# twosixlabs/csl-gan

Measured on AMD Instinct MI355X. Metric: images/sec/GPU CelebA DCResNet dp_mode=gc bs=128 at 1/2/4/8 MI355X, higher is better.
Workload: dtype f32; 1 GPU; CelebA DCResNet D-step: dp_mode=gc -gcm adaptive-pl -nms 32, WGAN-GP on mean samples, 3x64x64; compute_dtype=fp32_auto, storage_dtype=fp32, launch=hip_graph, batch_per_gpu=128, global_batch=128, parallelism=dp1, materialize=ghost, grad_sample_dtype=fp32, fuse_passes=True

## Files before the change

### csl_gan_amd/_lib.py

```python
from __future__ import annotations

import ctypes as C
import os

_HERE = os.path.dirname(os.path.abspath(__file__))
LIB_PATH = os.environ.get("CSLGAN_LIB_PATH") or os.path.join(_HERE, "libcslgan_hip.so")
MAX_SEGS = 16
ABI_VERSION = 7

EXPORTS = [
    "cslgan_version", "cslgan_last_error", "cslgan_last_kernel", "cslgan_device_count",
    "cslgan_sample_sqnorm_f32", "cslgan_sample_sqnorm_bf16", "cslgan_clip_factors_f32", "cslgan_clip_accum_noise_f32",
    "cslgan_clip_accum_noise_bf16", "cslgan_conv2d_wgrad_grouped_bf16out_f32",
    "cslgan_l2_clip_rows_f32", "cslgan_row_l2norm_f32", "cslgan_row_l2norm_bwd_f32", "cslgan_mean_sample_f32",
    "cslgan_conv2d_fwd_f32", "cslgan_conv2d_fwd_x3_f32", "cslgan_conv2d_dgrad_f32", "cslgan_conv2d_wgrad_grouped_f32",
    "cslgan_conv2d_wgrad_scaled_f32", "cslgan_conv2d_wgrad_blocks_f32", "cslgan_conv2d_wgrad_sqnorm_gram_f32", "cslgan_conv2d_wgrad_skinny_f32", "cslgan_conv2d_s2_fwd_f32",
    "cslgan_conv2d_dgrad_x3_f32", "cslgan_conv2d_s2_fwd_x3_f32", "cslgan_u8_to_f32_nhwc", "cslgan_split_filter_x3_f32",
    "cslgan_depth_to_space_f32", "cslgan_fold_channels4_f32",
    "cslgan_bias_grad_grouped_f32", "cslgan_act_bwd_f32", "cslgan_groupnorm_act_f32", "cslgan_groupnorm_apply_parts_f32", "cslgan_groupnorm_apply_parts_shortcut_f32", "cslgan_groupnorm_affine_parts_f32", "cslgan_batchnorm_act_f32", "cslgan_batchnorm_eval_act_f32",
    "cslgan_norm_act_bwd_f32", "cslgan_norm_bwd_ws_floats",
    "cslgan_adam_step_f32", "cslgan_adam_step_dev_f32", "cslgan_adam_multi_f32",
    "cslgan_adaptive_clip_f32", "cslgan_segment_means_f32", "cslgan_segment_means_bwd_f32", "cslgan_dstep_stats_f32", "cslgan_grad_log_stats_f32",
    "cslgan_lerp_rows_f32", "cslgan_lipschitz_term_f32", "cslgan_lipschitz_term_bwd_f32",
    "cslgan_conv2d_fwd_bf16s", "cslgan_conv2d_dgrad_bf16s", "cslgan_conv2d_wgrad_grouped_bf16s", "cslgan_cast_f32_bf16", "cslgan_cast_bf16_f32",
    "cslgan_act_bwd_bf16", "cslgan_bias_grad_grouped_bf16", "cslgan_linear_k1_dgrad_bf16s", "cslgan_linear_k1_wgrad_bf16s",
    "cslgan_conv2d_c3_fwd_bf16out", "cslgan_conv2d_c3_wgrad_bf16gy", "cslgan_groupnorm_act_bf16s",
    "cslgan_conv2d_fwd_skinny_bf16in", "cslgan_conv2d_dgrad_skinny_bf16in", "cslgan_conv2d_wgrad_scaled_bf16s",
    "cslgan_latent_normal_f32", "cslgan_f32_to_u8",
    "cslgan_attack_trials", "cslgan_rank_counts", "cslgan_softmax_max_rows_f32",
    "cslgan_ovr_logreg_ws_floats", "cslgan_ovr_logreg_eval_f32", "cslgan_ovr_logreg_proba_f32",
    "cslgan_ovr_logreg_u8_ws_floats", "cslgan_ovr_logreg_eval_u8", "cslgan_ovr_logreg_proba_u8",
    "cslgan_ovr_mlp_u8_ws_floats", "cslgan_ovr_mlp_eval_u8", "cslgan_ovr_mlp_proba_u8",
    "cslgan_class_moments_u8", "cslgan_nb_score_gauss_u8", "cslgan_nb_score_bern_u8",
    "cslgan_tree_best_split_ws_bytes", "cslgan_tree_best_split_u8", "cslgan_tree_apply_u8",
    "cslgan_boost_stump_ws_bytes", "cslgan_boost_stump_u8",
    "cslgan_nn_padded_dim", "cslgan_nn_prepare_u8", "cslgan_nn_min_i8", "cslgan_nn_count_i8",
    "cslgan_nn_kth_workspace_bytes", "cslgan_nn_kth_i8", "cslgan_nn_count_radius_i8",
    "cslgan_gram_d2_u8", "cslgan_svc_smo_f64",
    "cslgan_swd_directions_i8", "cslgan_swd_project_i8", "cslgan_sort_rows_ws_bytes", "cslgan_sort_rows_i32", "cslgan_swd_w1_i64",
]


class SegsT(C.Structure):
    _fields_ = [
        ("n_seg", C.c_int32), ("_pad", C.c_int32),
        ("inp", C.c_void_p * MAX_SEGS), ("out", C.c_void_p * MAX_SEGS), ("noise", C.c_void_p * MAX_SEGS),
        ("len", C.c_int64 * MAX_SEGS), ("row_stride", C.c_int64 * MAX_SEGS), ("rows", C.c_int64 * MAX_SEGS), ("call_counter", C.c_void_p),
    ]


MAX_CLIP_LAYERS, MAX_CLIP_JOBS = 32, 16


class AdaptiveClipT(C.Structure):
    _fields_ = [
        ("n_layers", C.c_int32), ("n_mat", C.c_int32), ("n_jobs", C.c_int32), ("_pad", C.c_int32),
        ("sq_adapt", C.c_void_p * MAX_CLIP_LAYERS), ("sq_rows", C.c_void_p * MAX_CLIP_LAYERS), ("mat_layer", C.c_int32 * MAX_CLIP_LAYERS),
        ("job_dst", C.c_void_p * MAX_CLIP_JOBS), ("job_first", C.c_int64 * MAX_CLIP_JOBS), ("job_layer", C.c_int32 * MAX_CLIP_JOBS),
        ("job_count", C.c_int32 * MAX_CLIP_JOBS), ("job_scale", C.c_float * MAX_CLIP_JOBS),
    ]


class ConvT(C.Structure):
    _fields_ = [(n, C.c_int32) for n in
                ("N", "H", "W", "C", "K", "R", "S", "stride", "pad", "compute", "P", "Q")] + [("split_ws", C.c_void_p), ("split_ws_floats", C.c_int64), ("gn_part", C.c_void_p), ("gn_groups", C.c_int32), ("in_relu", C.c_int32), ("in_scale", C.c_void_p), ("in_shift", C.c_void_p)]


_lib = None


class HipLibraryMissing(RuntimeError):
    pass


def lib():
    global _lib
    if _lib is not None:
        return _lib
    if not os.path.exists(LIB_PATH):
        raise HipLibraryMissing(
# ... 18 lines not shown
        "cslgan_row_l2norm_f32": [vp, i64, i64, vp, vp],
        "cslgan_row_l2norm_bwd_f32": [vp, vp, vp, i64, i64, vp, vp],
        "cslgan_conv2d_fwd_f32": [C.POINTER(ConvT), vp, vp, vp, vp, i32, vp, vp],
        "cslgan_conv2d_fwd_x3_f32": [C.POINTER(ConvT), vp, vp, vp, i32, vp, vp, i32, vp, vp],
        "cslgan_conv2d_dgrad_f32": [C.POINTER(ConvT), vp, vp, vp, i32, vp, vp, vp],
        "cslgan_conv2d_dgrad_x3_f32": [C.POINTER(ConvT), vp, vp, vp, vp, i32, vp, vp, vp],
        "cslgan_norm_act_bwd_f32": [vp, vp, vp, vp, vp, i64, i64, i32, i32, f32, i32, vp, vp, vp, vp, vp],
        "cslgan_depth_to_space_f32": [vp, i32, i32, i32, i32, i32, vp, vp],
        "cslgan_fold_channels4_f32": [vp, i64, i32, i32, vp, vp],
        "cslgan_conv2d_wgrad_grouped_f32": [C.POINTER(ConvT), vp, vp, i32, f32, vp, vp, vp],
        "cslgan_conv2d_wgrad_scaled_f32": [C.POINTER(ConvT), vp, vp, vp, i32, f32, vp, vp],
        "cslgan_conv2d_wgrad_blocks_f32": [C.POINTER(ConvT), vp, vp, f32, i32, C.POINTER(C.c_int32), C.POINTER(vp), C.POINTER(vp), vp],
        "cslgan_conv2d_wgrad_sqnorm_gram_f32": [C.POINTER(ConvT), vp, vp, f32, vp, vp],
        "cslgan_conv2d_wgrad_skinny_f32": [C.POINTER(ConvT), vp, vp, f32, vp, i32, vp],
        "cslgan_conv2d_s2_fwd_f32": [C.POINTER(ConvT), vp, vp, vp, i32, vp, i32, vp, vp],
        "cslgan_conv2d_s2_fwd_x3_f32": [C.POINTER(ConvT), vp, vp, vp, vp, i32, vp, i32, vp, vp],
        "cslgan_bias_grad_grouped_f32": [vp, i32, i32, i32, i32, f32, vp, vp, vp],
        "cslgan_act_bwd_f32": [vp, vp, i64, f32, vp, vp],
        "cslgan_groupnorm_act_f32": [vp, vp, vp, i32, i32, i32, i32, f32, i32, vp, vp, i32, vp, vp, vp],
        "cslgan_groupnorm_affine_parts_f32": [vp, i32, vp, vp, i32, i32, i32, i32, f32, vp, vp, vp],
        "cslgan_groupnorm_apply_parts_f32": [vp, vp, vp, i32, i32, i32, i32, f32, i32, vp, i32, vp, vp, i32, vp, vp],
        "cslgan_groupnorm_apply_parts_shortcut_f32": [vp, vp, vp, i32, i32, i32, i32, f32, i32, vp, i32, vp, vp, i32, vp, vp, i32, vp, vp],
        "cslgan_batchnorm_act_f32": [vp, vp, vp, i64, i32, f32, i32, f32, vp, vp, vp, vp, i64, i32, vp, vp, vp],
        "cslgan_batchnorm_eval_act_f32": [vp, vp, vp, vp, vp, i64, i32, f32, i32, vp, vp, i64, i32, vp, vp],
        "cslgan_adam_step_f32": [vp, vp, vp, vp, i64, f32, f32, f32, f32, f32, i32, vp],
        "cslgan_adam_step_dev_f32": [vp, vp, vp, vp, i64, f32, f32, f32, f32, f32, vp, vp],
        "cslgan_adam_multi_f32": [i32, C.POINTER(vp), C.POINTER(vp), C.POINTER(vp), C.POINTER(vp), C.POINTER(i64), f32, f32, f32, f32, f32,
                                  i32, vp, vp],
        "cslgan_adaptive_clip_f32": [C.POINTER(AdaptiveClipT), i64, i64, i32, f32, i32, f32, i64, vp, vp, vp, vp, vp, vp],
        "cslgan_segment_means_f32": [vp, i32, C.POINTER(C.c_int32), C.POINTER(f32), vp, vp, vp],
        "cslgan_segment_means_bwd_f32": [vp, vp, i32, C.POINTER(C.c_int32), C.POINTER(f32), vp, vp],
        "cslgan_dstep_stats_f32": [vp, i32, vp, i32, vp, vp, vp, vp, vp],
        "cslgan_grad_log_stats_f32": [vp, i32, i64, i64, i32, vp, i32, f32, vp, vp, vp, vp, vp, vp],
        "cslgan_lerp_rows_f32": [vp, vp, vp, i64, i64, vp, vp],
        "cslgan_lipschitz_term_f32": [vp, i64, i64, i32, f32, vp, vp, vp, vp, vp],
        "cslgan_lipschitz_term_bwd_f32": [vp, vp, vp, vp, i64, i64, i32, f32, vp, vp],
        "cslgan_conv2d_fwd_bf16s": [C.POINTER(ConvT), vp, vp, vp, i32, vp, vp, i32, i32, vp, i32, vp],
        "cslgan_conv2d_dgrad_bf16s": [C.POINTER(ConvT), vp, vp, vp, i32, vp, vp, i32, vp],
        "cslgan_conv2d_wgrad_grouped_bf16s": [C.POINTER(ConvT), vp, vp, i32, f32, vp, i32, vp, vp],
        "cslgan_cast_f32_bf16": [vp, vp, i64, vp],
        "cslgan_u8_to_f32_nhwc": [vp, vp, i32, i32, i32, i32, C.c_float, C.c_float, vp, vp],
        "cslgan_split_filter_x3_f32": [vp, i32, i32, i32, vp, i32, vp],
        "cslgan_cast_bf16_f32": [vp, vp, i64, vp],
        "cslgan_act_bwd_bf16": [vp, vp, i64, f32, vp, vp],
        "cslgan_bias_grad_grouped_bf16": [vp, i32, i32, i32, i32, f32, vp, vp, vp],
        "cslgan_linear_k1_dgrad_bf16s": [vp, vp, vp, i32, i64, vp, vp],
        "cslgan_linear_k1_wgrad_bf16s": [vp, vp, vp, i32, i64, i32, f32, vp, vp, vp],
        "cslgan_conv2d_wgrad_scaled_bf16s": [C.POINTER(ConvT), vp, vp, vp, i32, f32, vp, vp],
        "cslgan_conv2d_c3_fwd_bf16out": [C.POINTER(ConvT), vp, vp, vp, i32, vp, vp],
        "cslgan_conv2d_c3_wgrad_bf16gy": [C.POINTER(ConvT), vp, vp, f32, vp, vp, vp],
        "cslgan_groupnorm_act_bf16s": [vp, i32, vp, vp, i32, i32, i32, i32, f32, i32, vp, vp, i32, vp, vp],
        "cslgan_conv2d_fwd_skinny_bf16in": [C.POINTER(ConvT), vp, vp, vp, i32, vp, vp],
        "cslgan_conv2d_dgrad_skinny_bf16in": [C.POINTER(ConvT), vp, vp, vp, i32, vp, vp],
        "cslgan_latent_normal_f32": [u64, u64, vp, i64, i32, vp, i32, i32, vp, vp],
        "cslgan_f32_to_u8": [vp, i64, f32, f32, vp, vp],
        "cslgan_attack_trials": [vp, i64, vp, i64, i32, i32, u64, u64, i64, vp, vp],
        "cslgan_rank_counts": [vp, i64, vp, i64, vp, vp, vp],
        "cslgan_softmax_max_rows_f32": [vp, i64, i32, vp, vp],
        "cslgan_ovr_logreg_eval_f32": [vp, vp, vp, i64, i32, i32, vp, vp, vp, i64, vp],
        "cslgan_ovr_logreg_proba_f32": [vp, i32, vp, i64, i32, i32, vp, vp],
        "cslgan_ovr_logreg_eval_u8": [vp, vp, vp, i64, i32, i32, vp, vp, vp, i64, vp],
        "cslgan_ovr_logreg_proba_u8": [vp, vp, i64, i32, i32, vp, vp],
        "cslgan_ovr_mlp_eval_u8": [vp, vp, vp, i64, i32, i32, i32, f32, vp, vp, vp, vp],
        "cslgan_ovr_mlp_proba_u8": [vp, vp, i64, i32, i32, i32, vp, vp],
        "cslgan_class_moments_u8": [vp, vp, i64, i32, i32, i32, vp, vp, vp, vp, vp, vp],
        "cslgan_nb_score_gauss_u8": [vp, vp, vp, i64, i32, i32, vp, vp],
        "cslgan_nb_score_bern_u8": [vp, vp, i64, i32, i32, i32, vp, vp],
        "cslgan_tree_best_split_u8": [vp, vp, vp, i32, i64, i32, i32, vp, i64, vp, vp, vp, vp, vp, i64, C.c_uint32, u64, vp, vp, vp, i64, vp],
        "cslgan_tree_apply_u8": [vp, i64, i32, vp, vp, vp, vp, i32, i64, vp, vp],
        "cslgan_boost_stump_u8": [vp, vp, vp, i64, i32, i32, vp, vp, vp, i64, vp],
        "cslgan_nn_padded_dim": [i32],
        "cslgan_nn_prepare_u8": [vp, i64, i32, i32, vp, vp, vp],
        "cslgan_nn_min_i8": [vp, vp, i64, vp, vp, i64, i32, i64, vp, vp],
        "cslgan_nn_count_i8": [vp, vp, i64, vp, vp, i64, i32, vp, i32, vp, vp],
        "cslgan_nn_kth_i8": [vp, vp, i64, vp, vp, i64, i32, i64, i64, i32, vp, vp, i64, vp],
        "cslgan_nn_count_radius_i8": [vp, vp, i64, vp, vp, i64, i32, vp, vp, vp],
        "cslgan_gram_d2_u8": [vp, vp, i64, i32, vp, i64, vp],
        "cslgan_svc_smo_f64": [vp, i64, vp, i64, vp, vp, i32, C.c_double, C.c_double, i64, i64, vp, vp, vp, vp, vp],
        "cslgan_swd_directions_i8": [u64, i64, i32, i32, vp, vp],
        "cslgan_swd_project_i8": [vp, i64, vp, i64, i32, vp, i64, i64, vp],
        "cslgan_sort_rows_i32": [vp, i64, i64, i64, i32, vp, i64, vp],
        "cslgan_swd_w1_i64": [vp, i64, i64, vp, i64, i64, i64, vp, vp],
    }
    for name, args in sig.items():
        fn = getattr(L, name)
        fn.argtypes = args
        fn.restype = C.c_int
    L.cslgan_norm_bwd_ws_floats.argtypes = [i64, i64, i32, i32]
    L.cslgan_norm_bwd_ws_floats.restype = C.c_int64
    L.cslgan_ovr_logreg_ws_floats.argtypes = [i64, i32]
    L.cslgan_ovr_logreg_ws_floats.restype = C.c_int64
    L.cslgan_ovr_logreg_u8_ws_floats.argtypes = [i64, i32]
    L.cslgan_ovr_logreg_u8_ws_floats.restype = C.c_int64
    L.cslgan_ovr_mlp_u8_ws_floats.argtypes = [i64, i32, i32, i32]
    L.cslgan_ovr_mlp_u8_ws_floats.restype = C.c_int64
    L.cslgan_tree_best_split_ws_bytes.argtypes = [i64, i32]
    L.cslgan_tree_best_split_ws_bytes.restype = C.c_int64
    L.cslgan_boost_stump_ws_bytes.argtypes = [i32, i32]
    L.cslgan_boost_stump_ws_bytes.restype = C.c_int64
    L.cslgan_nn_kth_workspace_bytes.argtypes = [i64, i64, i32]
    L.cslgan_nn_kth_workspace_bytes.restype = C.c_int64
    L.cslgan_sort_rows_ws_bytes.argtypes = [i64, i64]
    L.cslgan_sort_rows_ws_bytes.restype = C.c_int64
    if L.cslgan_version() != ABI_VERSION:
        raise HipLibraryMissing("libcslgan_hip.so ABI version mismatch")
    _lib = L
# ... 8 lines not shown
```

### csl_gan_amd/build.py

```python
import os
import subprocess
import sys

HERE = os.path.dirname(os.path.abspath(__file__))
CSRC = os.path.join(HERE, "csrc")
LIB = os.path.join(HERE, "libcslgan_hip.so")
SOURCES = ["clip_kernels.hip", "igemm_kc.hip", "igemm_halo.hip", "igemm_skinny.hip", "igemm_mc.hip", "igemm_wgh.hip", "igemm_bf16.hip", "igemm_x3.hip", "igemm_bf16s.hip", "igemm_mcs.hip", "conv_c3.hip", "linear_k1.hip", "conv1x1.hip", "gn_shortcut.hip", "gram_norm.hip", "norm_kernels.hip", "layout_kernels.hip", "cast_kernels.hip", "step_kernels.hip", "attack_kernels.hip", "logreg_kernels.hip", "mlp_kernels.hip", "nb_kernels.hip", "tree_kernels.hip", "boost_kernels.hip", "nn_kernels.hip", "svm_kernels.hip", "swd_kernels.hip"]
HEADERS = ["common.h", "igemm.h", "conv_classes.h", "device_prims.h", "gn_apply.h", "kc_frame.h", "ovr_rows.h", "byte_split.h", "nn_tile.h", os.path.join("..", "..", "include", "cslgan.h")]


def _newer_than(target, deps):
    if not os.path.exists(target):
        return True
    t = os.path.getmtime(target)
    return any(os.path.getmtime(d) > t for d in deps)


def build(force=False, verbose=False):
    force = force or os.environ.get("CSLGAN_FORCE_BUILD", "0") == "1"
    hipcc = os.environ.get("HIPCC", "/opt/rocm/bin/hipcc")
    headers = [os.path.join(CSRC, h) for h in HEADERS]
    objs = []
    procs = []
    os.makedirs(os.path.join(HERE, "build"), exist_ok=True)
    jobs = int(os.environ.get("CSLGAN_BUILD_JOBS", str(min(8, os.cpu_count() or 1))))
    pending = []
    for s in SOURCES:
        o = os.path.join(HERE, "build", s.replace(".hip", ".o"))
        objs.append(o)
        if force or _newer_than(o, [os.path.join(CSRC, s)] + headers):
            pending.append((s, o))
    while pending or procs:
        while pending and len(procs) < jobs:
            s, o = pending.pop(0)
            cmd = [hipcc, "--offload-arch=gfx950", "-O3", "-fPIC", "-std=c++17", "-Wall", "-Wno-unused-function",
                   "-c", os.path.join(CSRC, s), "-o", o]
            if verbose:
                print(" ".join(cmd))
            procs.append((s, subprocess.Popen(cmd, stdout=subprocess.PIPE, stderr=subprocess.STDOUT)))
        s, pr = procs.pop(0)
        out, _ = pr.communicate()
        if pr.returncode != 0:
            for _, other in procs:
                other.kill()
            raise RuntimeError("hipcc failed on %s:\n%s" % (s, out.decode()))
        if verbose and out:
            print(out.decode())
    if not force and not _newer_than(LIB, objs):
        return LIB
    cmd = [hipcc, "--offload-arch=gfx950", "-shared", "-fPIC", "-o", LIB] + objs
    r = subprocess.run(cmd, stdout=subprocess.PIPE, stderr=subprocess.STDOUT)
    if r.returncode != 0:
        raise RuntimeError("link failed:\n" + r.stdout.decode())
    return LIB


if __name__ == "__main__":
    print(build(force="--force" in sys.argv, verbose=True))
```

### csl_gan_amd/csrc/igemm_skinny.hip

```cpp
#include "common.h"
#include "device_prims.h"
#include "igemm.h"
#include "conv_classes.h"

namespace cslgan {

constexpr int SK_MAXT = 9;
constexpr int SK_C = 64;
constexpr int SK_HALO = 12 * 12;

template <int NJ, bool ALL>
__global__ __launch_bounds__(256) void igemm_skinny_kernel(const KcParams p) {
    __shared__ float4 Hs[SK_HALO * 16];

    const int tid = threadIdx.x;
    const int b = xcd_remap(blockIdx.x, p.tiles_m);
    int ci = 0;
    if (!ALL) {
#pragma unroll 1
        while (ci + 1 < p.n_cls && b >= p.cls[ci + 1].tile0) ++ci;
    }
    const KcClass& kc = p.cls[ci];
    const int HW_ = kc.halo_w, hpix = kc.halo_h * kc.halo_w;
    const RowCoord rc0 = kc_decode_row((ALL ? b : b - kc.tile0) * 64, kc.OHc, kc.OWc, 1);
    const int y0 = rc0.oy + kc.ty_min, x0 = rc0.ox + kc.tx_min;
    const int img_base = rc0.img * p.AH * p.AW * SK_C;

    const __amdgpu_buffer_rsrc_t a_rsrc = make_rsrc(p.a, p.a_bytes);
    const int cl = tid & 15;
    if (p.a_bf16) {
        constexpr int HREG8 = (SK_HALO * 8 + 255) / 256;
        uint4 r8[HREG8];
#pragma unroll
        for (int j = 0; j < HREG8; ++j) {
            const int idx = tid + 256 * j;
            const int c8 = idx & 7, pix = idx >> 3;
            const int hy = pix / HW_, hx = pix - hy * HW_;
            const int iy = y0 + hy, ix = x0 + hx;
            const bool ok = pix < hpix && (unsigned)iy < (unsigned)p.VH && (unsigned)ix < (unsigned)p.VW;
            const auto v = buf_load4_raw(a_rsrc, (ok ? 2u * (unsigned)(img_base + (iy * p.AW + ix) * SK_C + c8 * 8) : BUF_OOB));
            r8[j] = make_uint4(v[0], v[1], v[2], v[3]);
        }
#pragma unroll
        for (int j = 0; j < HREG8; ++j) {
            const int idx = tid + 256 * j;
            if ((idx >> 3) < hpix) {
                const uint4 v = r8[j];
                Hs[2 * idx] = make_float4(bf_lo(v.x), bf_hi(v.x), bf_lo(v.y), bf_hi(v.y));
                Hs[2 * idx + 1] = make_float4(bf_lo(v.z), bf_hi(v.z), bf_lo(v.w), bf_hi(v.w));
            }
        }
    } else {
        constexpr int HREG = (SK_HALO * 16 + 255) / 256;
        float4 rh[HREG];
        unsigned okm = 0;
        const bool aff = p.in_scale != nullptr;
        float4 sc = make_float4(1.f, 1.f, 1.f, 1.f), sh = make_float4(0.f, 0.f, 0.f, 0.f);
        if (aff) {
            sc = *reinterpret_cast<const float4*>(p.in_scale + rc0.img * SK_C + cl * 4);
            sh = *reinterpret_cast<const float4*>(p.in_shift + rc0.img * SK_C + cl * 4);
        }
#pragma unroll
        for (int j = 0; j < HREG; ++j) {
            const int idx = tid + 256 * j;
            const int c4 = idx & 15, pix = idx >> 4;
// ... 30 lines not shown
    float4 wr[SK_MAXT][NJ];
    int toff[SK_MAXT];
#pragma unroll
    for (int t = 0; t < SK_MAXT; ++t) {
        toff[t] = t < Tc ? (((int)kk.ty[t] - kk.ty_min) * HW_ + ((int)kk.tx[t] - kk.tx_min)) * 16 : 0;
#pragma unroll
        for (int j = 0; j < NJ; ++j)
            wr[t][j] = buf_load4(w_rsrc, (t < Tc && j < p.Nn) ? 4u * (unsigned)(j * kk.Kdim + t * SK_C + cl * 4) : BUF_OOB);
    }
#pragma unroll
    for (int it = 0; it < 4; ++it) {
        const int q = wid * 16 + it * 4 + pg;
        const int qy = q >> 3, qx = q & 7;
        const int base = (qy * HW_ + qx) * 16 + cl;
        float acc[NJ];
#pragma unroll
        for (int j = 0; j < NJ; ++j) acc[j] = 0.f;
#pragma unroll
        for (int t = 0; t < SK_MAXT; ++t) {
            if (t < Tc) {
                const float4 a = Hs[base + toff[t]];
#pragma unroll
                for (int j = 0; j < NJ; ++j) {
                    acc[j] = fmaf(a.x, wr[t][j].x, acc[j]);
                    acc[j] = fmaf(a.y, wr[t][j].y, acc[j]);
                    acc[j] = fmaf(a.z, wr[t][j].z, acc[j]);
                    acc[j] = fmaf(a.w, wr[t][j].w, acc[j]);
                }
            }
        }
#pragma unroll
        for (int j = 0; j < NJ; ++j) {
            acc[j] += __shfl_xor(acc[j], 1);
            acc[j] += __shfl_xor(acc[j], 2);
            acc[j] += __shfl_xor(acc[j], 4);
            acc[j] += __shfl_xor(acc[j], 8);
        }
        if (cl < p.Nn) {
            float val = acc[0];
#pragma unroll
            for (int j = 1; j < NJ; ++j) val = cl == j ? acc[j] : val;
            val += bv;
            const RowCoord rc = {rc0.img, rc0.oy + qy, rc0.ox + qx};
            const int off = kc_out_offset(p, kk, rc);
            if (p.res) val += p.res[kc_res_offset(p, kk, rc) + cl];
            val = apply_act(val, p.act);
            if (p.mask) val = lrelu_mask(val, p.mask[off + cl]);
            p.out[off + cl] = val;
        }
    }
    }
}

bool skinny_eligible(const KcParams& p) {
    if (p.Nn > 4 || p.Nn < 1 || p.sy != 1 || p.sx != 1 || p.AC != SK_C) return false;
    if (!aligned16(p.a) || !aligned16(p.w)) return false;
    for (int c = 0; c < p.n_cls; ++c) {
        const KcClass& k = p.cls[c];
        if (k.T < 1 || k.T > SK_MAXT || (k.OHc & 7) || (k.OWc & 7) || (k.M & 63) || (k.w_off & 3)) return false;
        int ymin, ymax, xmin, xmax;
        tap_range(k, ymin, ymax, xmin, xmax);
        if (ymax - ymin > 4 || xmax - xmin > 4) return false;
    }
    return true;
}

int launch_skinny(KcParams& p, hipStream_t st) {
    int tm = 0;
    for (int c = 0; c < p.n_cls; ++c) {
        KcClass& k = p.cls[c];
        int ymin, ymax, xmin, xmax;
        tap_range(k, ymin, ymax, xmin, xmax);
        k.ty_min = ymin; k.tx_min = xmin; k.halo_h = 8 + ymax - ymin; k.halo_w = 8 + xmax - xmin;
        k.patch = 1;
        k.tile0 = tm;
        tm += k.M / 64;
    }
    bool all = p.n_cls > 1;
    int uy0 = 127, uy1 = -128, ux0 = 127, ux1 = -128;
    for (int c = 0; c < p.n_cls; ++c) {
        const KcClass& k = p.cls[c];
        all = all && k.OHc == p.cls[0].OHc && k.OWc == p.cls[0].OWc && k.M == p.cls[0].M;
        uy0 = k.ty_min < uy0 ? k.ty_min : uy0; ux0 = k.tx_min < ux0 ? k.tx_min : ux0;
        uy1 = k.ty_min + k.halo_h > uy1 ? k.ty_min + k.halo_h : uy1; ux1 = k.tx_min + k.halo_w > ux1 ? k.tx_min + k.halo_w : ux1;
    }
    all = all && (uy1 - uy0) * (ux1 - ux0) <= SK_HALO;
    if (all) {
        for (int c = 0; c < p.n_cls; ++c) {
            KcClass& k = p.cls[c];
            k.ty_min = uy0; k.tx_min = ux0; k.halo_h = uy1 - uy0; k.halo_w = ux1 - ux0;
        }
        tm = p.cls[0].M / 64;
    }
    p.tiles_m = tm;
    p.tiles_n = 1;
    p.ksplit = 1;
    const dim3 grid((unsigned)tm), block(256);
    note_kernel("igemm_skinny_kernel<%d%s>", p.Nn < 4 ? p.Nn : 4, all ? ",all" : "");
#define CSL_SKINNY(NJ_)                                                                              \
    if (all) hipLaunchKernelGGL((igemm_skinny_kernel<NJ_, true>), grid, block, 0, st, p);            \
    else hipLaunchKernelGGL((igemm_skinny_kernel<NJ_, false>), grid, block, 0, st, p);
    switch (p.Nn) {
        case 1: CSL_SKINNY(1) break;
        case 2: CSL_SKINNY(2) break;
        case 3: CSL_SKINNY(3) break;
        default: CSL_SKINNY(4) break;
    }
#undef CSL_SKINNY
    return check_launch("igemm_skinny_kernel");
}


struct SkinnyWgradParams {
    const float* gy;
    const float* x;
    int N, H, W, P, Q, T, n_patches;
    unsigned x_bytes;
    float alpha;
    float* partial;
    signed char ty[SK_MAXT], tx[SK_MAXT];
    int ty_min, tx_min, halo_h, halo_w;
};

template <int NJ>
__global__ __launch_bounds__(256) void skinny_wgrad_kernel(const SkinnyWgradParams p) {
    __shared__ float4 Hs[SK_HALO * 16];
    __shared__ float Gs[64 * 4];
    const int tid = threadIdx.x;
    const int T = p.T, HW_ = p.halo_w, hpix = p.halo_h * p.halo_w;
    const int cl = tid & 15, wid = tid >> 6, pg = (tid & 63) >> 4;
    const __amdgpu_buffer_rsrc_t x_rsrc = make_rsrc(p.x, p.x_bytes);
    int toff[SK_MAXT];
#pragma unroll
    for (int t = 0; t < SK_MAXT; ++t) toff[t] = t < T ? (((int)p.ty[t] - p.ty_min) * HW_ + ((int)p.tx[t] - p.tx_min)) * 16 : 0;
    float4 acc[SK_MAXT][NJ];
#pragma unroll
    for (int t = 0; t < SK_MAXT; ++t)
#pragma unroll
        for (int j = 0; j < NJ; ++j) acc[t][j] = make_float4(0.f, 0.f, 0.f, 0.f);

    constexpr int HREG = (SK_HALO * 16 + 255) / 256;
    const int per_img = (p.P >> 3) * (p.Q >> 3);
    for (int pt = blockIdx.x; pt < p.n_patches; pt += gridDim.x) {
        const int img = pt / per_img, rem = pt - img * per_img;
        const int gyy = rem / (p.Q >> 3), gxx = rem - gyy * (p.Q >> 3);
        const int oy0 = gyy << 3, ox0 = gxx << 3;
        float4 rh[HREG];
#pragma unroll
        for (int j = 0; j < HREG; ++j) {
            const int idx = tid + 256 * j;
            const int c4 = idx & 15, pix = idx >> 4;
            const int hy = pix / HW_, hx = pix - hy * HW_;
            const int iy = oy0 + p.ty_min + hy, ix = ox0 + p.tx_min + hx;
            const bool ok = pix < hpix && (unsigned)iy < (unsigned)p.H && (unsigned)ix < (unsigned)p.W;
            rh[j] = buf_load4(x_rsrc, ok ? 4u * (unsigned)(((img * p.H + iy) * p.W + ix) * SK_C + c4 * 4) : BUF_OOB);
        }
        float gv = 0.f;
        if (tid < 64 * NJ) {
            const int q = tid / NJ, j = tid - q * NJ;
// ... 5 lines not shown
            const int idx = tid + 256 * j;
            if ((idx >> 4) < hpix) Hs[idx] = rh[j];
        }
        if (tid < 64 * NJ) Gs[(tid / NJ) * 4 + (tid % NJ)] = gv;
        __syncthreads();
#pragma unroll
        for (int it = 0; it < 4; ++it) {
            const int q = wid * 16 + it * 4 + pg;
            const int base = ((q >> 3) * HW_ + (q & 7)) * 16 + cl;
            float g[NJ];
#pragma unroll
            for (int j = 0; j < NJ; ++j) g[j] = Gs[q * 4 + j];
#pragma unroll
            for (int t = 0; t < SK_MAXT; ++t) {
                if (t < T) {
                    const float4 a = Hs[base + toff[t]];
#pragma unroll
                    for (int j = 0; j < NJ; ++j) {
                        acc[t][j].x = fmaf(g[j], a.x, acc[t][j].x);
                        acc[t][j].y = fmaf(g[j], a.y, acc[t][j].y);
                        acc[t][j].z = fmaf(g[j], a.z, acc[t][j].z);
                        acc[t][j].w = fmaf(g[j], a.w, acc[t][j].w);
                    }
                }
            }
        }
    }
    __syncthreads();
    float* red = reinterpret_cast<float*>(Hs);
#pragma unroll
    for (int t = 0; t < SK_MAXT; ++t) {
        if (t < T) {
#pragma unroll
            for (int j = 0; j < NJ; ++j) {
                float4 v = acc[t][j];
                v.x += __shfl_xor(v.x, 16); v.y += __shfl_xor(v.y, 16); v.z += __shfl_xor(v.z, 16); v.w += __shfl_xor(v.w, 16);
                v.x += __shfl_xor(v.x, 32); v.y += __shfl_xor(v.y, 32); v.z += __shfl_xor(v.z, 32); v.w += __shfl_xor(v.w, 32);
                if (pg == 0) *reinterpret_cast<float4*>(&red[((wid * NJ + j) * T + t) * 64 + cl * 4]) = v;
            }
        }
    }
    __syncthreads();
    const int n_out = NJ * T * 64;
    float* dst = p.partial + (long long)blockIdx.x * n_out;
    for (int i = tid; i < n_out; i += 256)
        dst[i] = p.alpha * (red[i] + red[n_out + i] + red[2 * n_out + i] + red[3 * n_out + i]);
}

}

using namespace cslgan;

extern "C" {

int cslgan_conv2d_wgrad_skinny_f32(const cslgan_conv_t* c, const float* gy, const float* x, float alpha, float* partial,
                                   int n_blocks, void* stream) {
    CSLGAN_REQUIRE(c && gy && x && partial, "conv2d_wgrad_skinny: null argument");
    CSLGAN_REQUIRE(c->K >= 1 && c->K <= 4 && c->C == SK_C, "conv2d_wgrad_skinny: needs 1..4 output and 64 input channels");
    CSLGAN_REQUIRE(c->stride == 1 && c->R * c->S <= SK_MAXT && c->R <= 5 && c->S <= 5, "conv2d_wgrad_skinny: needs stride 1 and at most 9 taps");
    CSLGAN_REQUIRE(c->N > 0 && c->P == c->H + 2 * c->pad - c->R + 1 && c->Q == c->W + 2 * c->pad - c->S + 1, "conv2d_wgrad_skinny: inconsistent output size");
    CSLGAN_REQUIRE((c->P & 7) == 0 && (c->Q & 7) == 0, "conv2d_wgrad_skinny: output grid must be a multiple of 8x8");
    CSLGAN_REQUIRE(n_blocks >= 1 && aligned16(x), "conv2d_wgrad_skinny: bad workspace / alignment");
    CSLGAN_REQUIRE(4ll * c->N * c->H * c->W * SK_C < (long long)BUF_OOB, "conv2d_wgrad_skinny: input larger than 4 GB");
    SkinnyWgradParams p{};
    p.gy = gy; p.x = x; p.N = c->N; p.H = c->H; p.W = c->W; p.P = c->P; p.Q = c->Q; p.T = c->R * c->S;
    p.n_patches = c->N * (c->P >> 3) * (c->Q >> 3);
    p.x_bytes = (unsigned)(4ll * c->N * c->H * c->W * SK_C);
    p.alpha = alpha; p.partial = partial;
    fill_forward_taps(p.ty, p.tx, c->R, c->S, c->pad);
    p.ty_min = -c->pad; p.tx_min = -c->pad; p.halo_h = 8 + c->R - 1; p.halo_w = 8 + c->S - 1;
    const dim3 grid((unsigned)n_blocks), block(256);
    note_kernel("skinny_wgrad_kernel<%d>", c->K);
    switch (c->K) {
        case 1: hipLaunchKernelGGL((skinny_wgrad_kernel<1>), grid, block, 0, (hipStream_t)stream, p); break;
        case 2: hipLaunchKernelGGL((skinny_wgrad_kernel<2>), grid, block, 0, (hipStream_t)stream, p); break;
        case 3: hipLaunchKernelGGL((skinny_wgrad_kernel<3>), grid, block, 0, (hipStream_t)stream, p); break;
        default: hipLaunchKernelGGL((skinny_wgrad_kernel<4>), grid, block, 0, (hipStream_t)stream, p); break;
    }
    return check_launch("skinny_wgrad_kernel");
}

}
```

### include/cslgan.h

```cpp
#ifndef CSLGAN_H
#define CSLGAN_H

#include <stdint.h>

#ifdef __cplusplus
extern "C" {
#endif

#define CSLGAN_ABI_VERSION 7

typedef enum {
    CSLGAN_OK = 0,
    CSLGAN_ERR_INVALID_ARG = -1,
    CSLGAN_ERR_LAUNCH = -2,
    CSLGAN_ERR_NO_DEVICE = -3
} cslgan_status;

enum { CSLGAN_ACT_NONE = 0, CSLGAN_ACT_LRELU02 = 1, CSLGAN_ACT_RELU = 2, CSLGAN_ACT_TANH = 3 };

#define CSLGAN_MAX_SEGS 16
#define CSLGAN_MAX_ROLES 8

typedef struct {
    int32_t n_seg;
// ... 77 lines not shown
                                    float alpha, float* gw, float* sq, void* stream);

#define CSLGAN_MAX_WGRAD_BLOCKS 4
int cslgan_conv2d_wgrad_blocks_f32(const cslgan_conv_t* p, const float* gy, const float* x, float alpha, int n_blocks,
                                   const int32_t* block_first, float* const* gw, float* const* sq, void* stream);

int cslgan_conv2d_s2_fwd_f32(const cslgan_conv_t* p, const float* x, const float* w, float* wcls_ws, int repack,
                             const float* bias, int act, float* y, void* stream);

int cslgan_conv2d_s2_fwd_x3_f32(const cslgan_conv_t* p, const float* x, const float* w, float* wcls_ws, void* w3_ws, int repack,
                                const float* bias, int act, float* y, void* stream);

int cslgan_conv2d_wgrad_scaled_f32(const cslgan_conv_t* p, const float* gy, const float* x, const float* row_scale,
                                   int group, float alpha, float* gw, void* stream);

int cslgan_conv2d_wgrad_skinny_f32(const cslgan_conv_t* p, const float* gy, const float* x, float alpha, float* partial,
                                   int n_blocks, void* stream);

int cslgan_conv2d_wgrad_sqnorm_gram_f32(const cslgan_conv_t* p, const float* gy, const float* x, float alpha, float* sq,
                                        void* stream);

int cslgan_conv2d_wgrad_grouped_bf16out_f32(const cslgan_conv_t* p, const float* gy, const float* x, int group,
                                            float alpha, void* gw_bf16, float* sq, void* stream);

int cslgan_bias_grad_grouped_f32(const float* gy, int N, int PQ, int K, int group, float alpha,
                                 float* gb, float* sq, void* stream);


int cslgan_conv2d_fwd_bf16s(const cslgan_conv_t* p, const void* x, const float* w, void* wb_ws, int repack, const float* bias,
                            const void* residual, int res_bf16, int act, void* y, int y_bf16, void* stream);

int cslgan_conv2d_dgrad_bf16s(const cslgan_conv_t* p, const void* gy, const float* w, void* wt_ws, int repack, const void* mask,
                              void* gx, int gx_bf16, void* stream);

int cslgan_conv2d_wgrad_grouped_bf16s(const cslgan_conv_t* p, const void* gy, const void* x, int group, float alpha, void* gw,
                                      int gw_bf16, float* sq, void* stream);

int cslgan_linear_k1_dgrad_bf16s(const float* gy, const float* w, const void* mask_bf16, int N, int64_t C, void* gx_bf16, void* stream);
int cslgan_linear_k1_wgrad_bf16s(const float* gy, const void* x_bf16, const float* row_scale, int N, int64_t C, int group, float alpha,
                                 float* gw, float* sq, void* stream);

int cslgan_conv2d_c3_fwd_bf16out(const cslgan_conv_t* p, const float* x, const float* w, const float* bias, int act, void* y_bf16,
                                 void* stream);
int cslgan_conv2d_c3_wgrad_bf16gy(const cslgan_conv_t* p, const void* gy_bf16, const float* x, float alpha, float* gw, float* sq,
                                  void* stream);

int cslgan_groupnorm_act_bf16s(const void* x, int x_bf16, const float* gamma, const float* beta, int N, int HW, int C, int groups,
                               float eps, int relu, float* stats_ws, void* y_bf16, int d2s_W, void* x_shuffled_bf16, void* stream);

int cslgan_conv2d_fwd_skinny_bf16in(const cslgan_conv_t* p, const void* x_bf16, const float* w, const float* bias, int act, float* y,
                                    void* stream);
int cslgan_conv2d_dgrad_skinny_bf16in(const cslgan_conv_t* p, const void* gy_bf16, const float* w, float* wt_ws, int repack, float* gx,
                                      void* stream);

int cslgan_conv2d_wgrad_scaled_bf16s(const cslgan_conv_t* p, const void* gy, const void* x, const float* row_scale, int group, float alpha,
                                     float* gw, void* stream);

int cslgan_cast_f32_bf16(const float* in, void* out_bf16, int64_t n, void* stream);
int cslgan_cast_bf16_f32(const void* in_bf16, float* out, int64_t n, void* stream);

int cslgan_act_bwd_bf16(const void* g, const void* y, int64_t n, float slope, void* out, void* stream);
int cslgan_bias_grad_grouped_bf16(const void* gy, int N, int PQ, int K, int group, float alpha, float* gb, float* sq, void* stream);


int cslgan_act_bwd_f32(const float* g, const float* y, int64_t n, float slope, float* out, void* stream);

int cslgan_depth_to_space_f32(const float* in, int N, int H, int W, int C, int inverse, float* out, void* stream);
int cslgan_fold_channels4_f32(const float* in, int64_t rows, int C, int unfold, float* out, void* stream);

#define CSLGAN_NORM_PARTIAL_BLOCKS 64
int cslgan_groupnorm_affine_parts_f32(const float* part, int n_part, const float* gamma, const float* beta, int N, int HW, int C, int groups,
                                      float eps, float* scale, float* shift, void* stream);
int cslgan_groupnorm_apply_parts_f32(const float* x, const float* gamma, const float* beta, int N, int HW, int C, int groups,
                                     float eps, int relu, const float* part, int n_part, float* stats_ws, float* y, int d2s_W,
                                     float* x_shuffled, void* stream);
int cslgan_groupnorm_act_f32(const float* x, const float* gamma, const float* beta, int N, int HW, int C,
                             int groups, float eps, int relu, float* stats_ws, float* y, int d2s_W, float* x_shuffled,
                             float* scratch, void* stream);
int cslgan_groupnorm_apply_parts_shortcut_f32(const float* x, const float* gamma, const float* beta, int N, int HW, int C, int groups,
                                              float eps, int relu, const float* part, int n_part, float* stats_ws, float* y,
                                              int d2s_W, const float* wf, const float* bias, int K, float* s, void* stream);

int cslgan_batchnorm_act_f32(const float* x, const float* gamma, const float* beta, int64_t rows, int C, float eps,
                             int relu, float momentum, float* running_mean, float* running_var, float* stats_ws,
                             float* y, int64_t rows_per_image, int d2s_W, float* x_shuffled, float* scratch ,
                             void* stream);

int cslgan_batchnorm_eval_act_f32(const float* x, const float* gamma, const float* beta, const float* running_mean,
                                  const float* running_var, int64_t rows, int C, float eps, int relu, float* stats_ws,
                                  float* y, int64_t rows_per_image, int d2s_W, float* x_shuffled, void* stream);

int cslgan_norm_act_bwd_f32(const float* x, const float* dy, const float* y, const float* gamma, const float* stats,
                            int64_t rows, int64_t rows_per_stat, int C, int groups, float eps, int relu, float* ws,
                            float* dx, float* dgamma, float* dbeta, void* stream);
int64_t cslgan_norm_bwd_ws_floats(int64_t rows, int64_t rows_per_stat, int C, int groups);

int cslgan_adam_step_f32(float* p, const float* g, float* m, float* v, int64_t n, float lr, float b1,
                         float b2, float eps, float weight_decay, int step, void* stream);
int cslgan_adam_step_dev_f32(float* p, const float* g, float* m, float* v, int64_t n, float lr, float b1,
                             float b2, float eps, float weight_decay, const int32_t* step_dev, void* stream);

int cslgan_adam_multi_f32(int n_seg, float* const* p, const float* const* g, float* const* m, float* const* v, const int64_t* n,
                          float lr, float b1, float b2, float eps, float weight_decay, int step, const int32_t* step_dev,
                          void* stream);

int cslgan_segment_means_f32(const float* x, int n_seg, const int32_t* sizes, const float* scale, float* vec, float* total,
// ... 116 lines not shown
```

Measured before the change: 20520 images/sec.

## Make skinny conv kernel persistent over patch runs with prefetched halos

Adds a new skinny conv kernel in which each block processes a run of consecutive 8x8 output patches. It keeps the filter in registers, or in LDS when all classes are handled together, and prefetches the next patch's halo into registers while computing the current one. Pixel dot products use packed FMA and DPP cross-lane reductions. The aim is to amortize filter loads and block launch costs and to hide global-load latency. The old per-patch kernel is kept as a fallback for Nn=4, for large LDS needs and when a runtime knob disables runs. The trade-off is dynamic LDS use and fewer blocks, which risks lower occupancy and load imbalance.

```diff
diff --git a/csl_gan_amd/_lib.py b/csl_gan_amd/_lib.py
--- a/csl_gan_amd/_lib.py
+++ b/csl_gan_amd/_lib.py
@@ -25,7 +25,7 @@
     "cslgan_conv2d_fwd_bf16s", "cslgan_conv2d_dgrad_bf16s", "cslgan_conv2d_wgrad_grouped_bf16s", "cslgan_cast_f32_bf16", "cslgan_cast_bf16_f32",
     "cslgan_act_bwd_bf16", "cslgan_bias_grad_grouped_bf16", "cslgan_linear_k1_dgrad_bf16s", "cslgan_linear_k1_wgrad_bf16s",
     "cslgan_conv2d_c3_fwd_bf16out", "cslgan_conv2d_c3_wgrad_bf16gy", "cslgan_groupnorm_act_bf16s",
-    "cslgan_conv2d_fwd_skinny_bf16in", "cslgan_conv2d_dgrad_skinny_bf16in", "cslgan_conv2d_wgrad_scaled_bf16s",
+    "cslgan_conv2d_fwd_skinny_bf16in", "cslgan_conv2d_dgrad_skinny_bf16in", "cslgan_conv2d_wgrad_scaled_bf16s", "cslgan_skinny_run_length",
     "cslgan_latent_normal_f32", "cslgan_f32_to_u8",
     "cslgan_attack_trials", "cslgan_rank_counts", "cslgan_softmax_max_rows_f32",
     "cslgan_ovr_logreg_ws_floats", "cslgan_ovr_logreg_eval_f32", "cslgan_ovr_logreg_proba_f32",
@@ -150,6 +150,7 @@
         "cslgan_groupnorm_act_bf16s": [vp, i32, vp, vp, i32, i32, i32, i32, f32, i32, vp, vp, i32, vp, vp],
         "cslgan_conv2d_fwd_skinny_bf16in": [C.POINTER(ConvT), vp, vp, vp, i32, vp, vp],
         "cslgan_conv2d_dgrad_skinny_bf16in": [C.POINTER(ConvT), vp, vp, vp, i32, vp, vp],
+        "cslgan_skinny_run_length": [i32],
         "cslgan_latent_normal_f32": [u64, u64, vp, i64, i32, vp, i32, i32, vp, vp],
         "cslgan_f32_to_u8": [vp, i64, f32, f32, vp, vp],
         "cslgan_attack_trials": [vp, i64, vp, i64, i32, i32, u64, u64, i64, vp, vp],
diff --git a/csl_gan_amd/build.py b/csl_gan_amd/build.py
--- a/csl_gan_amd/build.py
+++ b/csl_gan_amd/build.py
@@ -6,7 +6,7 @@
 CSRC = os.path.join(HERE, "csrc")
 LIB = os.path.join(HERE, "libcslgan_hip.so")
 SOURCES = ["clip_kernels.hip", "igemm_kc.hip", "igemm_halo.hip", "igemm_skinny.hip", "igemm_mc.hip", "igemm_wgh.hip", "igemm_bf16.hip", "igemm_x3.hip", "igemm_bf16s.hip", "igemm_mcs.hip", "conv_c3.hip", "linear_k1.hip", "conv1x1.hip", "gn_shortcut.hip", "gram_norm.hip", "norm_kernels.hip", "layout_kernels.hip", "cast_kernels.hip", "step_kernels.hip", "attack_kernels.hip", "logreg_kernels.hip", "mlp_kernels.hip", "nb_kernels.hip", "tree_kernels.hip", "boost_kernels.hip", "nn_kernels.hip", "svm_kernels.hip", "swd_kernels.hip"]
-HEADERS = ["common.h", "igemm.h", "conv_classes.h", "device_prims.h", "gn_apply.h", "kc_frame.h", "ovr_rows.h", "byte_split.h", "nn_tile.h", os.path.join("..", "..", "include", "cslgan.h")]
+HEADERS = ["common.h", "igemm.h", "conv_classes.h", "skinny_runs.h", "device_prims.h", "gn_apply.h", "kc_frame.h", "ovr_rows.h", "byte_split.h", "nn_tile.h", os.path.join("..", "..", "include", "cslgan.h")]
 
 
 def _newer_than(target, deps):
diff --git a/csl_gan_amd/csrc/igemm_skinny.hip b/csl_gan_amd/csrc/igemm_skinny.hip
--- a/csl_gan_amd/csrc/igemm_skinny.hip
+++ b/csl_gan_amd/csrc/igemm_skinny.hip
@@ -1,16 +1,22 @@
+#include <atomic>
 #include "common.h"
 #include "device_prims.h"
 #include "igemm.h"
 #include "conv_classes.h"
+#include "skinny_runs.h"
 
 namespace cslgan {
 
 constexpr int SK_MAXT = 9;
 constexpr int SK_C = 64;
 constexpr int SK_HALO = 12 * 12;
+constexpr int SK_CUS = 256;
+constexpr unsigned SK_LDS_MAX = 64u * 1024u;
+
+static std::atomic<int> g_skinny_run_length{-1};
 
 template <int NJ, bool ALL>
-__global__ __launch_bounds__(256) void igemm_skinny_kernel(const KcParams p) {
+__global__ __launch_bounds__(256) void igemm_skinny_patch_kernel(const KcParams p) {
     __shared__ float4 Hs[SK_HALO * 16];
 
     const int tid = threadIdx.x;
@@ -147,6 +153,252 @@
     }
 }
 
+template <int NJ>
+__device__ __forceinline__ void sk_pair_filter(const float4 (&w)[NJ], float4 (&q)[NJ]) {
+    if (NJ == 1) q[0] = w[0];
+    if (NJ >= 2) {
+        q[0] = make_float4(w[0].x, w[NJ >= 2 ? 1 : 0].x, w[0].y, w[NJ >= 2 ? 1 : 0].y);
+        q[NJ >= 2 ? 1 : 0] = make_float4(w[0].z, w[NJ >= 2 ? 1 : 0].z, w[0].w, w[NJ >= 2 ? 1 : 0].w);
+    }
+    if (NJ == 3) q[NJ - 1] = w[NJ - 1];
+}
+
+template <int CTRL>
+__device__ __forceinline__ float sk_dpp(float v) {
+    return __builtin_bit_cast(float, __builtin_amdgcn_update_dpp(0, __builtin_bit_cast(int, v), CTRL, 0xF, 0xF, true));
+}
+
+template <int NJ, int T>
+__device__ __forceinline__ void sk_pixels(const float4* Hs, int base0, int HW_, const int (&toff)[SK_MAXT], const float4 (&wq)[SK_MAXT][NJ],
+                                          float (&acc)[4][NJ], int Tc = T) {
+    constexpr int O = NJ - 1;
+#pragma unroll
+    for (int it = 0; it < 4; ++it) {
+        const int base = base0 + ((it >> 1) * HW_ + (it & 1) * 4) * 16;
+        f32x2 ap = {0.f, 0.f};
+        float as = 0.f;
+        float4 ah[T > 0 ? T : 1];
+        if (T > 0) {
+#pragma unroll
+            for (int t = 0; t < T; ++t) ah[t] = Hs[base + toff[t]];
+            __builtin_amdgcn_sched_barrier(0);
+        }
+#pragma unroll
+        for (int t = 0; t < (T > 0 ? T : SK_MAXT); ++t) {
+            if (T > 0 || t < Tc) {
+                const float4 a = T > 0 ? ah[T > 0 ? t : 0] : Hs[base + toff[t]];
+                if (NJ >= 2) {
+                    const float4 w01 = wq[t][0], w23 = wq[t][NJ >= 2 ? 1 : 0];
+                    ap = __builtin_elementwise_fma(f32x2{a.x, a.x}, f32x2{w01.x, w01.y}, ap);
+                    ap = __builtin_elementwise_fma(f32x2{a.y, a.y}, f32x2{w01.z, w01.w}, ap);
+                    ap = __builtin_elementwise_fma(f32x2{a.z, a.z}, f32x2{w23.x, w23.y}, ap);
+                    ap = __builtin_elementwise_fma(f32x2{a.w, a.w}, f32x2{w23.z, w23.w}, ap);
+                }
+                if (NJ & 1) {
+                    const float4 w = wq[t][O];
+                    as = fmaf(a.x, w.x, as);
+                    as = fmaf(a.y, w.y, as);
+                    as = fmaf(a.z, w.z, as);
+                    as = fmaf(a.w, w.w, as);
+                }
+            }
+        }
+        if (NJ >= 2) { acc[it][0] = ap.x; acc[it][NJ >= 2 ? 1 : 0] = ap.y; }
+        if (NJ & 1) acc[it][O] = as;
+        asm volatile("" : "+v"(base0) : "v"(acc[it][0]));
+    }
+#pragma unroll
+    for (int it = 0; it < 4; ++it)
+#pragma unroll
+        for (int j = 0; j < NJ; ++j) {
+            acc[it][j] += sk_dpp<0xB1>(acc[it][j]);
+            acc[it][j] += sk_dpp<0x4E>(acc[it][j]);
+            acc[it][j] += sk_dpp<0x141>(acc[it][j]);
+            acc[it][j] += sk_dpp<0x140>(acc[it][j]);
+        }
+}
+
+extern __shared__ float4 sk_lds[];
+
+template <int NJ, bool ALL>
+__global__ __launch_bounds__(256, 2) void igemm_skinny_kernel(const KcParams p, const SkinnyRuns runs) {
+    constexpr int HREG = (SK_HALO * 16 + 255) / 256;
+    constexpr int HREG8 = (SK_HALO * 8 + 255) / 256;
+
+    const int tid = threadIdx.x;
+    const SkinnyRun run = skinny_run_at(runs, xcd_remap(blockIdx.x, skinny_grid(runs)));
+    const int ci = ALL ? 0 : run.cls;
+    const KcClass& kc = p.cls[ci];
+    const int HW_ = kc.halo_w, hpix = kc.halo_h * kc.halo_w;
+    const unsigned hw_rcp = (65536u + (unsigned)HW_ - 1u) / (unsigned)HW_;
+    const int nslot = (hpix + 15) >> 4, nslot8 = (hpix + 31) >> 5;
+    float4* const Hs = sk_lds;
+    float4* const Ws = sk_lds + hpix * 16;
+
+    const __amdgpu_buffer_rsrc_t a_rsrc = make_rsrc(p.a, p.a_bytes);
+    const int cl = tid & 15, wid = tid >> 6, pg = (tid & 63) >> 4;
+    const bool aff = !ALL && p.in_scale != nullptr && !p.a_bf16;
+    const float aff_lo = p.in_relu ? 0.f : -__builtin_inff();
+
+    u32x4 rr[HREG];
+    unsigned okm = 0;
+    float4 sc = make_float4(1.f, 1.f, 1.f, 1.f), sh = make_float4(0.f, 0.f, 0.f, 0.f);
+    const int gsh = p.a_bf16 ? 3 : 4;
+    const int nsl = p.a_bf16 ? nslot8 : nslot;
+    const __amdgpu_buffer_rsrc_t sc_rsrc = make_rsrc(p.in_scale, aff ? 0x7FFFFFF0u : 0u), sh_rsrc = make_rsrc(p.in_shift, aff ? 0x7FFFFFF0u : 0u);
+    auto fetch = [&](int i) {
+        const bool live = i < run.n;
+        const RowCoord rc0 = kc_decode_row((run.patch0 + i) * 64, kc.OHc, kc.OWc, 1);
+        const int y0 = rc0.oy + kc.ty_min, x0 = rc0.ox + kc.tx_min;
+        const int img_base = rc0.img * p.AH * p.AW * SK_C;
+        okm = 0;
+        int tid_ = tid;
+        asm volatile("" : "+v"(tid_));
+        if (!ALL) {
+            const unsigned tab = live ? 4u * (unsigned)(rc0.img * SK_C + cl * 4) : BUF_OOB;
+            sc = buf_load4(sc_rsrc, tab);
+            sh = buf_load4(sh_rsrc, tab);
+        }
+#pragma unroll
+        for (int j = 0; j < HREG; ++j) {
+            if (j < nsl) {
+                const int idx = tid_ + 256 * j;
+                const int cg = idx & ((1 << gsh) - 1), pix = idx >> gsh;
+                const int hy = (int)(__umul24((unsigned)pix, hw_rcp) >> 16), hx = pix - __mul24(hy, HW_);
+                const int iy = y0 + hy, ix = x0 + hx;
+                const bool ok = live && pix < hpix && (unsigned)iy < (unsigned)p.VH && (unsigned)ix < (unsigned)p.VW;
+                okm |= (ok ? 1u : 0u) << j;
+                const unsigned elem = (unsigned)(img_base + ((__mul24(iy, p.AW) + ix) << 6) + (cg << (6 - gsh)));
+                rr[j] = buf_load4_raw(a_rsrc, ok ? (elem << (p.a_bf16 ? 1 : 2)) : BUF_OOB);
+            }
+        }
+    };
+    auto commit = [&]() {
+        if (p.a_bf16) {
+#pragma unroll
+            for (int j = 0; j < HREG8; ++j) {
+                const int idx = tid + 256 * j;
+                if (j < nslot8 && (idx >> 3) < hpix) {
+                    const u32x4 v = rr[j];
+                    Hs[2 * idx] = make_float4(bf_lo(v.x), bf_hi(v.x), bf_lo(v.y), bf_hi(v.y));
+                    Hs[2 * idx + 1] = make_float4(bf_lo(v.z), bf_hi(v.z), bf_lo(v.w), bf_hi(v.w));
+                }
+            }
+        } else {
+#pragma unroll
+            for (int j = 0; j < HREG; ++j) {
+                const int idx = tid + 256 * j;
+                if (j < nslot) {
+                    float4 v = make_float4(__uint_as_float(rr[j].x), __uint_as_float(rr[j].y), __uint_as_float(rr[j].z), __uint_as_float(rr[j].w));
+                    if (aff) {
+                        const bool in = (okm >> j) & 1u;
+                        v.x = in ? fmaxf(fmaf(sc.x, v.x, sh.x), aff_lo) : 0.f;
+                        v.y = in ? fmaxf(fmaf(sc.y, v.y, sh.y), aff_lo) : 0.f;
+                        v.z = in ? fmaxf(fmaf(sc.z, v.z, sh.z), aff_lo) : 0.f;
+                        v.w = in ? fmaxf(fmaf(sc.w, v.w, sh.w), aff_lo) : 0.f;
+                    }
+                    if ((idx >> 4) < hpix) Hs[idx] = v;
+                }
+            }
+        }
+    };
+
+    fetch(0);
+
+    float4 wr[SK_MAXT][NJ];
+    if (ALL) {
+        int lo = 0;
+#pragma unroll 1
+        for (int c = 0; c < p.n_cls; ++c) {
+            const KcClass& kk = p.cls[c];
+            const int n4 = (p.Nn * kk.Kdim) >> 2;
+            const __amdgpu_buffer_rsrc_t w_rsrc = make_rsrc(p.w + kk.w_off, p.w_bytes - 4u * (unsigned)kk.w_off);
+            for (int i = tid; i < kk.T * 16; i += 256) {
+                float4 w[NJ], q[NJ];
+#pragma unroll
+                for (int j = 0; j < NJ; ++j) w[j] = buf_load4(w_rsrc, 4u * (unsigned)(j * kk.Kdim + i * 4));
+                sk_pair_filter<NJ>(w, q);
+#pragma unroll
+                for (int j = 0; j < NJ; ++j) Ws[lo + i * NJ + j] = q[j];
+            }
+            lo += n4;
+        }
+    } else {
+        const __amdgpu_buffer_rsrc_t w_rsrc = make_rsrc(p.w + kc.w_off, p.w_bytes - 4u * (unsigned)kc.w_off);
+#pragma unroll
+        for (int t = 0; t < SK_MAXT; ++t) {
+            float4 w[NJ];
+#pragma unroll
+            for (int j = 0; j < NJ; ++j)
+                w[j] = buf_load4(w_rsrc, (t < kc.T && j < p.Nn) ? 4u * (unsigned)(j * kc.Kdim + t * SK_C + cl * 4) : BUF_OOB);
+            sk_pair_filter<NJ>(w, wr[t]);
+        }
+    }
+    const int e_it = cl / NJ, e_j = cl - e_it * NJ;
+    const bool e_on = cl < 4 * NJ;
+    float bv = 0.f;
+    if (p.bias && e_on) bv = p.bias[e_j];
+    asm volatile("" : : "v"(bv));
+    if (!ALL) {
+#pragma unroll
+        for (int t = 0; t < SK_MAXT; ++t)
+#pragma unroll
+            for (int j = 0; j < NJ; ++j) asm volatile("" : : "v"(wr[t][j].x), "v"(wr[t][j].y), "v"(wr[t][j].z), "v"(wr[t][j].w));
+    }
+
+#pragma unroll 1
+    for (int i = 0; i < runs.R; ++i) {
+        commit();
+        __syncthreads();
+        const bool live = i < run.n;
+        const RowCoord rc0 = kc_decode_row((run.patch0 + i) * 64, kc.OHc, kc.OWc, 1);
+        if (i + 1 < runs.R) fetch(i + 1);
+
+        int lo = 0;
+#pragma unroll 1
+        for (int cc = ALL ? 0 : ci; cc < (ALL ? p.n_cls : ci + 1); ++cc) {
+            const KcClass& kk = p.cls[cc];
+            const int Tc = kk.T;
+            int toff[SK_MAXT];
+#pragma unroll
+            for (int t = 0; t < SK_MAXT; ++t) {
+                toff[t] = t < Tc ? (((int)kk.ty[t] - kk.ty_min) * HW_ + ((int)kk.tx[t] - kk.tx_min)) * 16 : 0;
+                if (ALL) {
+#pragma unroll
+                    for (int j = 0; j < NJ; ++j)
+                        wr[t][j] = t < Tc ? Ws[lo + (t * 16 + cl) * NJ + j] : make_float4(0.f, 0.f, 0.f, 0.f);
+                }
+            }
+            lo += (p.Nn * kk.Kdim) >> 2;
+            float acc[4][NJ];
+            int base0 = (wid * 2 * HW_ + pg) * 16 + cl;
+            asm volatile("" : "+v"(base0));
+            switch (Tc) {
+                case 9: sk_pixels<NJ, 9>(Hs, base0, HW_, toff, wr, acc); break;
+                case 6: sk_pixels<NJ, 6>(Hs, base0, HW_, toff, wr, acc); break;
+                case 4: sk_pixels<NJ, 4>(Hs, base0, HW_, toff, wr, acc); break;
+                default: sk_pixels<NJ, 0>(Hs, base0, HW_, toff, wr, acc, Tc); break;
+            }
+            if (live && e_on) {
+                float val = acc[0][0];
+#pragma unroll
+                for (int it = 0; it < 4; ++it)
+#pragma unroll
+                    for (int j = 0; j < NJ; ++j) val = cl == it * NJ + j ? acc[it][j] : val;
+                val += bv;
+                const int q = wid * 16 + e_it * 4 + pg;
+                const RowCoord rc = {rc0.img, rc0.oy + (q >> 3), rc0.ox + (q & 7)};
+                const int off = kc_out_offset(p, kk, rc);
+                if (p.res) val += p.res[kc_res_offset(p, kk, rc) + e_j];
+                val = apply_act(val, p.act);
+                if (p.mask) val = lrelu_mask(val, p.mask[off + e_j]);
+                p.out[off + e_j] = val;
+            }
+        }
+        __syncthreads();
+    }
+}
+
 bool skinny_eligible(const KcParams& p) {
     if (p.Nn > 4 || p.Nn < 1 || p.sy != 1 || p.sx != 1 || p.AC != SK_C) return false;
     if (!aligned16(p.a) || !aligned16(p.w)) return false;
@@ -190,16 +442,42 @@
     p.tiles_m = tm;
     p.tiles_n = 1;
     p.ksplit = 1;
-    const dim3 grid((unsigned)tm), block(256);
-    note_kernel("igemm_skinny_kernel<%d%s>", p.Nn < 4 ? p.Nn : 4, all ? ",all" : "");
-#define CSL_SKINNY(NJ_)                                                                              \
-    if (all) hipLaunchKernelGGL((igemm_skinny_kernel<NJ_, true>), grid, block, 0, st, p);            \
-    else hipLaunchKernelGGL((igemm_skinny_kernel<NJ_, false>), grid, block, 0, st, p);
+    const dim3 block(256);
+    int patches[SKR_MAX_CLS] = {0, 0, 0, 0}, hpix_max = 0;
+    unsigned w_floats = 0;
+    for (int c = 0; c < p.n_cls; ++c) {
+        const KcClass& k = p.cls[c];
+        patches[c] = k.M / 64;
+        hpix_max = k.halo_h * k.halo_w > hpix_max ? k.halo_h * k.halo_w : hpix_max;
+        w_floats += (unsigned)(p.Nn * k.Kdim);
+    }
+    const unsigned lds = 256u * (unsigned)hpix_max + (all ? 4u * w_floats : 0u);
+    const int mode = g_skinny_run_length.load(std::memory_order_relaxed);
+    if (mode == 0 || lds > SK_LDS_MAX || p.Nn > 3 || (all && p.in_scale)) {
+        const dim3 grid((unsigned)tm);
+        note_kernel("igemm_skinny_patch_kernel<%d%s>", p.Nn < 4 ? p.Nn : 4, all ? ",all" : "");
+#define CSL_SKINNY(NJ_)                                                                                    \
+    if (all) hipLaunchKernelGGL((igemm_skinny_patch_kernel<NJ_, true>), grid, block, 0, st, p);            \
+    else hipLaunchKernelGGL((igemm_skinny_patch_kernel<NJ_, false>), grid, block, 0, st, p);
+        switch (p.Nn) {
+            case 1: CSL_SKINNY(1) break;
+            case 2: CSL_SKINNY(2) break;
+            case 3: CSL_SKINNY(3) break;
+            default: CSL_SKINNY(4) break;
+        }
+#undef CSL_SKINNY
+        return check_launch("igemm_skinny_patch_kernel");
+    }
+    const SkinnyRuns runs = skinny_plan_runs(patches, all ? 1 : p.n_cls, mode > 0 ? mode : skinny_run_length(tm, SK_CUS));
+    const dim3 grid((unsigned)skinny_grid(runs));
+    note_kernel("igemm_skinny_kernel<%d%s>", p.Nn, all ? ",all" : "");
+#define CSL_SKINNY(NJ_)                                                                                    \
+    if (all) hipLaunchKernelGGL((igemm_skinny_kernel<NJ_, true>), grid, block, lds, st, p, runs);          \
+    else hipLaunchKernelGGL((igemm_skinny_kernel<NJ_, false>), grid, block, lds, st, p, runs);
     switch (p.Nn) {
         case 1: CSL_SKINNY(1) break;
         case 2: CSL_SKINNY(2) break;
-        case 3: CSL_SKINNY(3) break;
-        default: CSL_SKINNY(4) break;
+        default: CSL_SKINNY(3) break;
     }
 #undef CSL_SKINNY
     return check_launch("igemm_skinny_kernel");
@@ -311,6 +589,11 @@
 using namespace cslgan;
 
 extern "C" {
+
+int cslgan_skinny_run_length(int patches) {
+    g_skinny_run_length.store(patches < 0 ? -1 : patches > SKR_MAX_RUN ? SKR_MAX_RUN : patches, std::memory_order_relaxed);
+    return CSLGAN_OK;
+}
 
 int cslgan_conv2d_wgrad_skinny_f32(const cslgan_conv_t* c, const float* gy, const float* x, float alpha, float* partial,
                                    int n_blocks, void* stream) {
diff --git a/csl_gan_amd/csrc/skinny_runs.h b/csl_gan_amd/csrc/skinny_runs.h
--- /dev/null
+++ b/csl_gan_amd/csrc/skinny_runs.h
@@ -0,0 +1,61 @@
+#pragma once
+#include <stdint.h>
+
+#ifndef CSL_HD
+#if defined(__HIPCC__)
+#define CSL_HD __host__ __device__ __forceinline__
+#else
+#define CSL_HD inline
+#endif
+#endif
+
+namespace cslgan {
+
+constexpr int SKR_MAX_CLS = 4;
+constexpr int SKR_MAX_RUN = 16;
+constexpr int SKR_RUNS_PER_CU = 4;
+
+struct SkinnyRuns {
+    int R, n_cls;
+    int patches[SKR_MAX_CLS];
+    int run0[SKR_MAX_CLS + 1];
+};
+struct SkinnyRun {
+    int cls;
+    int patch0;
+    int n;
+};
+
+CSL_HD int skinny_run_length(long long patches, int n_cu) {
+    const long long r = patches / ((long long)SKR_RUNS_PER_CU * (n_cu > 0 ? n_cu : 1));
+    return r < 1 ? 1 : r > SKR_MAX_RUN ? SKR_MAX_RUN : (int)r;
+}
+
+CSL_HD SkinnyRuns skinny_plan_runs(const int* patches, int n_cls, int R) {
+    SkinnyRuns s;
+    s.R = R < 1 ? 1 : R > SKR_MAX_RUN ? SKR_MAX_RUN : R;
+    s.n_cls = n_cls < 1 ? 1 : n_cls > SKR_MAX_CLS ? SKR_MAX_CLS : n_cls;
+    s.run0[0] = 0;
+    for (int c = 0; c < SKR_MAX_CLS; ++c) {
+        s.patches[c] = (c < s.n_cls && patches[c] > 0) ? patches[c] : 0;
+        s.run0[c + 1] = s.run0[c] + (s.patches[c] + s.R - 1) / s.R;
+    }
+    return s;
+}
+
+CSL_HD int skinny_grid(const SkinnyRuns& s) { return s.n_cls <= 1 ? s.run0[1] : s.n_cls == 2 ? s.run0[2] : s.n_cls == 3 ? s.run0[3] : s.run0[4]; }
+
+CSL_HD SkinnyRun skinny_run_at(const SkinnyRuns& s, int r) {
+    int c = 0, first = s.run0[0], patches = s.patches[0];
+    if (s.n_cls > 1 && r >= s.run0[1]) { c = 1; first = s.run0[1]; patches = s.patches[1]; }
+    if (s.n_cls > 2 && r >= s.run0[2]) { c = 2; first = s.run0[2]; patches = s.patches[2]; }
+    if (s.n_cls > 3 && r >= s.run0[3]) { c = 3; first = s.run0[3]; patches = s.patches[3]; }
+    SkinnyRun u;
+    u.cls = c;
+    u.patch0 = (r - first) * s.R;
+    const int left = patches - u.patch0;
+    u.n = left < s.R ? left : s.R;
+    return u;
+}
+
+}
diff --git a/include/cslgan.h b/include/cslgan.h
--- a/include/cslgan.h
+++ b/include/cslgan.h
@@ -153,6 +153,7 @@
                                     void* stream);
 int cslgan_conv2d_dgrad_skinny_bf16in(const cslgan_conv_t* p, const void* gy_bf16, const float* w, float* wt_ws, int repack, float* gx,
                                       void* stream);
+int cslgan_skinny_run_length(int patches);
 
 int cslgan_conv2d_wgrad_scaled_bf16s(const cslgan_conv_t* p, const void* gy, const void* x, const float* row_scale, int group, float alpha,
                                      float* gw, void* stream);
```

Measured after the change: 20580 images/sec (median of 6 runs). Within noise of the previous version (+0.3%).
